# ishine/minimax-speech

Measured on AMD Instinct MI355X. Metric: 24 kHz audio-seconds generated per wall-second per node (CosyVoice2-0.5B-shaped LM + flow + DAC-VAE, end to end), higher is better.
Workload: dtype bf16

## Files before the change

include/mmx_hip_lab.h:

```cpp
#ifndef MMX_HIP_LAB_H
#define MMX_HIP_LAB_H
#ifdef __cplusplus
extern "C" {
#endif

int mmx_lab_skinny_stamps(void* buf);

int mmx_lab_tail_stamps(void* buf);

#ifdef __cplusplus
}
#endif
#endif
```

minimax-speech_amd/csrc/llm.hip:

```cpp
#include "common.h"
#include "../../include/mmx_hip.h"

template <typename T>
__global__ void pack_skinny_kernel(const T* __restrict__ w, long ldw, int N, int K, const float* __restrict__ kscale,
                                   int half, T* __restrict__ wp) {
    constexpr int E = sizeof(T) == 2 ? 8 : 4;
    constexpr int KB = E * 4;
    const long total = (long)((N + 15) / 16) * (K / KB) * 64 * E;
    for (long idx = (long)blockIdx.x * blockDim.x + threadIdx.x; idx < total; idx += (long)gridDim.x * blockDim.x) {
        int j = idx % E;
        long t = idx / E;
        int lane = t % 64;
        t /= 64;
        int kb = t % (K / KB);
        int tile = t / (K / KB);
        int col = lane & 15, g = lane >> 4;
        int row;
        if (half > 0) row = (tile & 1) * half + (tile >> 1) * 16 + col;
        else row = tile * 16 + col;
        int kk = kb * KB + g * E + j;
        float v = 0.f;
        if (row < N && (half == 0 || ((tile >> 1) * 16 + col) < half)) {
            v = Cvt<T>::to_f(w[(long)row * ldw + kk]);
            if (kscale) v *= kscale[kk];
// ... 343 lines not shown
                               const int32_t* __restrict__ block_table, int max_pages, int page) {
    constexpr int D = 64, HALF = 32;
    const int b = blockIdx.y, t = blockIdx.x;
    const int p = pos[b] + t;
    const float* src = qkv + (long)b * qkv_bs + (long)t * ldqkv;
    const int nh = Hq + 2 * Hkv;
    const int phys = block_table[(long)b * max_pages + p / page];
    const int slot = p % page;
    for (int i = threadIdx.x; i < nh * HALF; i += blockDim.x) {
        const int hh = i / HALF, d = i % HALF;
        const float x0 = src[hh * D + d], x1 = src[hh * D + d + HALF];
        float y0 = x0, y1 = x1;
        if (hh < Hq + Hkv) {
            const float ang = (float)p * inv_freq[d];
            const float c = cosf(ang), s = sinf(ang);
            y0 = x0 * c - x1 * s;
            y1 = x1 * c + x0 * s;
        }
        if (hh < Hq) {
            T* o = q_out + (long)b * q_bs + (long)t * ldq + hh * D;
            o[d] = Cvt<T>::from_f(y0);
            o[d + HALF] = Cvt<T>::from_f(y1);
        } else {
            const int hk = (hh - Hq) % Hkv;
            T* base = (hh < Hq + Hkv ? kc : vc) + (((long)phys * Hkv + hk) * page + slot) * D;
            base[d] = Cvt<T>::from_f(y0);
            base[d + HALF] = Cvt<T>::from_f(y1);
        }
    }
}
extern "C" int mmx_rope_kv_store(const float* qkv, int64_t ldqkv, int64_t qkv_bs, int B, int rows, int Hq, int Hkv, int D,
                                 const float* inv_freq, const int32_t* pos, void* q_out, int64_t ldq, int64_t q_bs,
                                 void* kc, void* vc, const int32_t* block_table, int max_pages, int page,
                                 int dtype, hipStream_t stream) {
    dtype = MMX_ACT_DTYPE(dtype);
    MMX_CHECK_ARG(qkv && inv_freq && pos && q_out && kc && vc && block_table && B > 0 && rows > 0 && D == 64 && page > 0);
    dim3 grid(rows, B);
    if (dtype == MMX_BF16) hipLaunchKernelGGL(rope_kv_kernel<bf16_t>, grid, dim3(256), 0, stream, qkv, ldqkv, qkv_bs, Hq, Hkv, inv_freq, pos, (bf16_t*)q_out, ldq, q_bs, (bf16_t*)kc, (bf16_t*)vc, block_table, max_pages, page);
    else if (dtype == MMX_F32) hipLaunchKernelGGL(rope_kv_kernel<float>, grid, dim3(256), 0, stream, qkv, ldqkv, qkv_bs, Hq, Hkv, inv_freq, pos, (float*)q_out, ldq, q_bs, (float*)kc, (float*)vc, block_table, max_pages, page);
    else return MMX_EARG;
    MMX_LAUNCH_CHECK();
    return MMX_OK;
}

template <typename T>
__global__ __launch_bounds__(256) void paged_attn_kernel(
    const T* __restrict__ q, long ldq, long q_bs, int Hq, int Hkv, float scale, const int32_t* __restrict__ pos,
    const T* __restrict__ kc, const T* __restrict__ vc, const int32_t* __restrict__ block_table, int max_pages,
    int page, T* __restrict__ out, long ldo, long o_bs) {
    constexpr int D = 64;
    extern __shared__ __attribute__((aligned(16))) char smem[];
    float* qs = reinterpret_cast<float*>(smem);
    float* red = qs + D;
    float* S = red + 8 + 4 * D;
    const int tid = threadIdx.x, lane = tid & 63, wave = tid >> 6;
    const int h = blockIdx.x, t = blockIdx.y, b = blockIdx.z;
    const int hk = h / (Hq / Hkv);
    const int ctx = pos[b] + t + 1;
    const int32_t* bt = block_table + (long)b * max_pages;
    if (tid < D) qs[tid] = Cvt<T>::to_f(q[(long)b * q_bs + (long)t * ldq + h * D + tid]);
    __syncthreads();
    float mx = -INFINITY;
    for (int j = tid; j < ctx; j += 256) {
        const T* kp = kc + (((long)bt[j / page] * Hkv + hk) * page + j % page) * D;
        float s = 0.f;
#pragma unroll
        for (int d = 0; d < D; ++d) s += qs[d] * Cvt<T>::to_f(kp[d]);
        s *= scale;
        S[j] = s;
        mx = fmaxf(mx, s);
    }
    mx = wave_max(mx);
    if (lane == 0) red[wave] = mx;
    __syncthreads();
    mx = fmaxf(fmaxf(red[0], red[1]), fmaxf(red[2], red[3]));
    float l = 0.f;
    for (int j = tid; j < ctx; j += 256) {
        float e = expf(S[j] - mx);
        S[j] = e;
        l += e;
    }
    l = wave_sum(l);
    if (lane == 0) red[4 + wave] = l;
    __syncthreads();
    l = red[4] + red[5] + red[6] + red[7];
    float acc = 0.f;
    for (int j = wave; j < ctx; j += 4) {
        const T* vp = vc + (((long)bt[j / page] * Hkv + hk) * page + j % page) * D;
        acc += S[j] * Cvt<T>::to_f(vp[lane]);
    }
    red[8 + wave * D + lane] = acc;
    __syncthreads();
    if (wave == 0) {
        float o = (red[8 + lane] + red[8 + D + lane]) + (red[8 + 2 * D + lane] + red[8 + 3 * D + lane]);
        out[(long)b * o_bs + (long)t * ldo + h * D + lane] = Cvt<T>::from_f(o / l);
    }
}
extern "C" int mmx_paged_attn(const void* q, int64_t ldq, int64_t q_bs, int B, int rows, int Hq, int Hkv, int D, float scale,
                              const int32_t* pos, const void* kc, const void* vc, const int32_t* block_table, int max_pages,
                              int page, void* out, int64_t ldo, int64_t o_bs, int dtype, hipStream_t stream) {
    dtype = MMX_ACT_DTYPE(dtype);
    MMX_CHECK_ARG(q && pos && kc && vc && block_table && out && B > 0 && rows > 0 && D == 64 && Hq % Hkv == 0 && page > 0);
    const size_t max_ctx = (size_t)max_pages * page;
    size_t lds = (64 + 8 + 4 * 64 + max_ctx) * 4;
    MMX_CHECK_ARG(lds <= 160 * 1024);
    dim3 grid(Hq, rows, B);
    if (dtype == MMX_BF16) MMX_LDS_OPT_IN(paged_attn_kernel<bf16_t>, lds);
    else if (dtype == MMX_F32) MMX_LDS_OPT_IN(paged_attn_kernel<float>, lds);
    if (dtype == MMX_BF16) hipLaunchKernelGGL(paged_attn_kernel<bf16_t>, grid, dim3(256), lds, stream, (const bf16_t*)q, ldq, q_bs, Hq, Hkv, scale, pos, (const bf16_t*)kc, (const bf16_t*)vc, block_table, max_pages, page, (bf16_t*)out, ldo, o_bs);
    else if (dtype == MMX_F32) hipLaunchKernelGGL(paged_attn_kernel<float>, grid, dim3(256), lds, stream, (const float*)q, ldq, q_bs, Hq, Hkv, scale, pos, (const float*)kc, (const float*)vc, block_table, max_pages, page, (float*)out, ldo, o_bs);
    else return MMX_EARG;
    MMX_LAUNCH_CHECK();
    return MMX_OK;
}

template <typename T>
__device__ __forceinline__ void load8(const T* p, float o[8]) {
    if constexpr (sizeof(T) == 2) {
        uint4 r = *reinterpret_cast<const uint4*>(p);
        const unsigned w[4] = {r.x, r.y, r.z, r.w};
#pragma unroll
        for (int i = 0; i < 4; ++i) {
            o[2 * i] = __uint_as_float(w[i] << 16);
            o[2 * i + 1] = __uint_as_float(w[i] & 0xffff0000u);
        }
    } else {
        float4 a = *reinterpret_cast<const float4*>(p), b = *reinterpret_cast<const float4*>(p + 4);
        o[0] = a.x; o[1] = a.y; o[2] = a.z; o[3] = a.w; o[4] = b.x; o[5] = b.y; o[6] = b.z; o[7] = b.w;
    }
}
template <typename T>
struct Raw8 {
    uint4 a, b;
    __device__ __forceinline__ void load(const T* p) {
        a = *reinterpret_cast<const uint4*>(p);
        if constexpr (sizeof(T) == 4) b = *reinterpret_cast<const uint4*>(p + 4);
    }
    __device__ __forceinline__ void to_float(float o[8]) const {
        const unsigned w[4] = {a.x, a.y, a.z, a.w};
        if constexpr (sizeof(T) == 2) {
#pragma unroll
            for (int i = 0; i < 4; ++i) {
                o[2 * i] = __uint_as_float(w[i] << 16);
                o[2 * i + 1] = __uint_as_float(w[i] & 0xffff0000u);
            }
        } else {
            const unsigned w2[4] = {b.x, b.y, b.z, b.w};
#pragma unroll
            for (int i = 0; i < 4; ++i) { o[i] = __uint_as_float(w[i]); o[4 + i] = __uint_as_float(w2[i]); }
        }
    }
};

template <typename T, int OM, int HP>
__global__ __launch_bounds__(256) void decode_attn_kernel(
    const float* __restrict__ qkv, long ldqkv, int Hq, int Hkv, const float* __restrict__ inv_freq,
    const float* __restrict__ rope_tab, const int32_t* __restrict__ pos, T* __restrict__ kc, T* __restrict__ vc,
    const int32_t* __restrict__ block_table, int max_pages, int page, float scale, T* __restrict__ out, long ldo,
    int nseq) {
    constexpr int D = 64, HALF = 32, NG = 32;
    extern __shared__ __attribute__((aligned(16))) char smem[];
    float* qs = reinterpret_cast<float*>(smem);
    float* kn = qs + HP * D;
    float* vn = kn + D;
    float* gm = vn + D;
    float* gl = gm + HP * NG;
    float* part = gl + HP * NG;
    int* bts = reinterpret_cast<int*>(part + HP * NG * D);
    const int tid = threadIdx.x;
    const int group = Hq / Hkv, nsub = (group + HP - 1) / HP;
    const int xcd = blockIdx.x & 7, slot = blockIdx.x >> 3;
    const int kvg = (slot / nsub) * 8 + xcd;
    if (kvg >= Hkv * nseq) return;
    const int b = kvg / Hkv, hk = kvg % Hkv, sub = slot % nsub;
    const int h0 = hk * group + sub * HP, nh = min(HP, group - sub * HP);
    const int32_t* bt = block_table + (long)b * max_pages;
    for (int i = tid; i < max_pages; i += 256) bts[i] = bt[i];
    const int p = pos[b];
    const float* src = qkv + (long)b * ldqkv;
    const float sc2 = scale * 1.44269504088896341f;
    if (tid < (HP + 1) * HALF) {
        const int which = tid >> 5, d = tid & 31;
        const float* x = src + (which < HP ? (h0 + min(which, nh - 1)) * D : (Hq + hk) * D);
        float c, s;
        if (rope_tab) {
            c = rope_tab[(long)p * D + d];
            s = rope_tab[(long)p * D + HALF + d];
        } else {
            const float ang = (float)p * inv_freq[d];
            c = cosf(ang);
            s = sinf(ang);
        }
        const float y0 = x[d] * c - x[d + HALF] * s, y1 = x[d + HALF] * c + x[d] * s;
        if (which < HP) { qs[which * D + d] = y0 * sc2; qs[which * D + d + HALF] = y1 * sc2; }
        else { kn[d] = Cvt<T>::to_f(Cvt<T>::from_f(y0)); kn[d + HALF] = Cvt<T>::to_f(Cvt<T>::from_f(y1)); }
    } else if (tid < (HP + 1) * HALF + D) {
        const int d = tid - (HP + 1) * HALF;
        vn[d] = Cvt<T>::to_f(Cvt<T>::from_f(src[(Hq + Hkv + hk) * D + d]));
    }
    __syncthreads();
    if (sub == 0 && tid < D) {
        const long o = (((long)bts[p / page] * Hkv + hk) * page + p % page) * D + tid;
        kc[o] = Cvt<T>::from_f(kn[tid]);
        vc[o] = Cvt<T>::from_f(vn[tid]);
    }
    const int kg = tid >> 3, dc = tid & 7;
    float qv[HP][8];
#pragma unroll
    for (int hp = 0; hp < HP; ++hp)
#pragma unroll
        for (int e = 0; e < 8; ++e) qv[hp][e] = qs[hp * D + dc * 8 + e];
    float m[HP], l[HP], acc[HP][8];
#pragma unroll
    for (int hp = 0; hp < HP; ++hp) {
        m[hp] = -INFINITY;
        l[hp] = 0.f;
#pragma unroll
        for (int e = 0; e < 8; ++e) acc[hp][e] = 0.f;
    }
    auto consume = [&](const float kv[8], const float vv[8]) {
#pragma unroll
        for (int hp = 0; hp < HP; ++hp) {
            float sdot = 0.f;
#pragma unroll
            for (int e = 0; e < 8; ++e) sdot = __builtin_fmaf(qv[hp][e], kv[e], sdot);
            sdot = group8_sum(sdot);
            const float mn = fmaxf(m[hp], sdot);
            const float al = __builtin_amdgcn_exp2f(m[hp] - mn), pj = __builtin_amdgcn_exp2f(sdot - mn);
            l[hp] = __builtin_fmaf(l[hp], al, pj);
#pragma unroll
            for (int e = 0; e < 8; ++e) acc[hp][e] = __builtin_fmaf(acc[hp][e], al, pj * vv[e]);
            m[hp] = mn;
        }
    };
    constexpr int U = sizeof(T) == 2 ? 12 : 10;
    for (int j0 = kg; j0 < p; j0 += NG * U) {
        Raw8<T> rk[U], rv[U];
#pragma unroll
        for (int u = 0; u < U; ++u) {
            const int j = j0 + u * NG;
            if (j < p) {
                const long o = (((long)bts[j / page] * Hkv + hk) * page + j % page) * D + dc * 8;
                rk[u].load(kc + o);
                rv[u].load(vc + o);
            }
        }
#pragma unroll
        for (int u = 0; u < U; ++u) {
            if (j0 + u * NG < p) {
                float kv[8], vv[8];
                rk[u].to_float(kv);
                rv[u].to_float(vv);
                consume(kv, vv);
            }
        }
    }
    if (kg == p % NG) {
        float kv[8], vv[8];
#pragma unroll
        for (int e = 0; e < 8; ++e) { kv[e] = kn[dc * 8 + e]; vv[e] = vn[dc * 8 + e]; }
        consume(kv, vv);
    }
#pragma unroll
    for (int hp = 0; hp < HP; ++hp) {
        if (dc == 0) { gm[hp * NG + kg] = m[hp]; gl[hp * NG + kg] = l[hp]; }
#pragma unroll
        for (int e = 0; e < 8; ++e) part[(hp * NG + kg) * D + dc * 8 + e] = acc[hp][e];
    }
    __syncthreads();
    if (tid < nh * D) {
        const int hp = tid >> 6, d = tid & 63, h = h0 + hp;
        const float* gmh = gm + hp * NG;
        const float* glh = gl + hp * NG;
        const float* ph = part + hp * NG * D;
        float M = -INFINITY;
#pragma unroll
        for (int g2 = 0; g2 < NG; ++g2) M = fmaxf(M, gmh[g2]);
        float L = 0.f, o = 0.f;
#pragma unroll
        for (int g2 = 0; g2 < NG; ++g2) {
            const float w = __builtin_amdgcn_exp2f(gmh[g2] - M);
            L = __builtin_fmaf(glh[g2], w, L);
            o = __builtin_fmaf(ph[g2 * D + d], w, o);
        }
        if constexpr (OM == 2) {
            const int nkb = Hq * D / 32, col = h * D + d;
            const long ps = (long)((nseq + 15) / 16) * nkb * 512;
            const long idx = ((((long)(b >> 4) * nkb + (col >> 5)) * 64) + (((col & 31) >> 3) << 4) + (b & 15)) * 8 + (col & 7);
            bf16_t* pl = reinterpret_cast<bf16_t*>(out);
            const float v = o / L;
            const bf16_t hh = f2bf(v);
            const float r1 = v - bf2f(hh);
            const bf16_t mm = f2bf(r1);
            pl[idx] = hh;
            pl[ps + idx] = mm;
            pl[2 * ps + idx] = f2bf(r1 - bf2f(mm));
        } else if constexpr (OM == 3) {
            const int nkb = Hq * D / 32, col = h * D + d;
            const long ps = (long)((nseq + 15) / 16) * nkb * 512;
            const long idx = ((((long)(b >> 4) * nkb + (col >> 5)) * 64) + (((col & 31) >> 3) << 4) + (b & 15)) * 8 + (col & 7);
            unsigned short* pl = reinterpret_cast<unsigned short*>(out);
            const float v = o / L;
            const _Float16 hh = (_Float16)v;
            pl[idx] = __builtin_bit_cast(unsigned short, hh);
            pl[ps + idx] = __builtin_bit_cast(unsigned short, (_Float16)(v - (float)hh));
        } else {
            out[OM == 1 ? act_packed_index<T>(b, h * D + d, Hq * D) : (long)b * ldo + h * D + d] = Cvt<T>::from_f(o / L);
        }
    }
}

template <bool OPK, int G>
__global__ __launch_bounds__(256) void decode_attn_gqa_kernel(
    const float* __restrict__ qkv, long ldqkv, int Hq, int Hkv, const float* __restrict__ inv_freq,
    const float* __restrict__ rope_tab, const int32_t* __restrict__ pos, bf16_t* __restrict__ kc, bf16_t* __restrict__ vc,
    const int32_t* __restrict__ block_table, int max_pages, float scale, bf16_t* __restrict__ out, long ldo, int nseq) {
    constexpr int D = 64, HALF = 32, PAGE = 16, NS = 8;
    static_assert(G <= 8, "one 8-float row of P per key");
    extern __shared__ __attribute__((aligned(16))) char smem[];
    bf16_t* qh = reinterpret_cast<bf16_t*>(smem);
    bf16_t* ql = qh + 16 * D;
    bf16_t* kn = ql + 16 * D;
    bf16_t* vn = kn + D;
    float* Pw = reinterpret_cast<float*>(vn + D);
    float* Aw = Pw + 4 * NS * 16 * 8;
    float* gm = Aw + 32;
    float* gl = gm + 32;
    float* part = gl + 32;
    int* bts = reinterpret_cast<int*>(part + 32 * G * D);
    const int tid = threadIdx.x, wave = tid >> 6, lane = tid & 63, l16 = lane & 15, g = lane >> 4;
    const int b = blockIdx.x / Hkv, hk = blockIdx.x % Hkv;
    const int32_t* bt = block_table + (long)b * max_pages;
    const int p = pos[b];
    const int NT = p / PAGE + 1;
    for (int i = tid; i < NT; i += 256) bts[i] = bt[i];
    for (int i = tid; i < 2 * 16 * D / 2; i += 256) reinterpret_cast<unsigned*>(qh)[i] = 0u;
    __syncthreads();
    const float* src = qkv + (long)b * ldqkv;
    const float sc2 = scale * 1.44269504088896341f;
    {
        const int which = tid >> 5, d = tid & 31;
        if (which <= G) {
            const float* x = src + (which < G ? (hk * G + which) * D : (Hq + hk) * D);
            float c, s;
            if (rope_tab) {
                c = rope_tab[(long)p * D + d];
                s = rope_tab[(long)p * D + HALF + d];
            } else {
                const float ang = (float)p * inv_freq[d];
                c = cosf(ang);
                s = sinf(ang);
            }
            const float y0 = x[d] * c - x[d + HALF] * s, y1 = x[d + HALF] * c + x[d] * s;
            if (which < G) {
                const float a0 = y0 * sc2, a1 = y1 * sc2;
                const bf16_t h0 = f2bf(a0), h1 = f2bf(a1);
                qh[which * D + d] = h0;
                qh[which * D + d + HALF] = h1;
                ql[which * D + d] = f2bf(a0 - bf2f(h0));
                ql[which * D + d + HALF] = f2bf(a1 - bf2f(h1));
            } else {
                kn[d] = f2bf(y0);
                kn[d + HALF] = f2bf(y1);
            }
        }
        if (tid < D) vn[tid] = f2bf(src[(Hq + Hkv + hk) * D + tid]);
    }
    __syncthreads();
    if (tid < D) {
        const long o = (((long)bts[p / PAGE] * Hkv + hk) * PAGE + p % PAGE) * D + tid;
        kc[o] = kn[tid];
        vc[o] = vn[tid];
    }
    short8_t bqh[2], bql[2];
#pragma unroll
    for (int ks = 0; ks < 2; ++ks) {
        bqh[ks] = *reinterpret_cast<const short8_t*>(qh + l16 * D + ks * 32 + 8 * g);
        bql[ks] = *reinterpret_cast<const short8_t*>(ql + l16 * D + ks * 32 + 8 * g);
    }
    const int ksub = lane >> 3, dc = lane & 7;
    const int tp = p / PAGE, rp = p % PAGE;
    float* Pme = Pw + wave * NS * 16 * 8;
    float m_run = -INFINITY, l_part = 0.f;
    typedef __attribute__((ext_vector_type(2))) float float2_t;
    float2_t acc[G][4];
#pragma unroll
    for (int h = 0; h < G; ++h)
#pragma unroll
        for (int e = 0; e < 4; ++e) acc[h][e] = float2_t{0.f, 0.f};

    for (int r0 = 0; r0 < NT; r0 += 4 * NS) {
        if (r0 + wave >= NT) break;
        uint4 rk[NS][2], rv[NS][2];
#pragma unroll
        for (int i = 0; i < NS; ++i) {
            const int t = r0 + 4 * i + wave;
            if (t < NT) {
                const long base = ((long)bts[t] * Hkv + hk) * PAGE * D;
#pragma unroll
                for (int ks = 0; ks < 2; ++ks) rk[i][ks] = *reinterpret_cast<const uint4*>(kc + base + l16 * D + ks * 32 + 8 * g);
#pragma unroll
                for (int hf = 0; hf < 2; ++hf) rv[i][hf] = *reinterpret_cast<const uint4*>(vc + base + (ksub + 8 * hf) * D + dc * 8);
            }
        }
        float4_t sacc[NS];
        float bm = -INFINITY;
#pragma unroll
        for (int i = 0; i < NS; ++i) {
            const int t = r0 + 4 * i + wave;
            sacc[i] = float4_t{-INFINITY, -INFINITY, -INFINITY, -INFINITY};
            if (t < NT) {
                if (t == tp) {
                    if (l16 == rp) {
#pragma unroll
                        for (int ks = 0; ks < 2; ++ks) rk[i][ks] = *reinterpret_cast<const uint4*>(kn + ks * 32 + 8 * g);
                    }
#pragma unroll
                    for (int hf = 0; hf < 2; ++hf) {
                        if (ksub + 8 * hf == rp) rv[i][hf] = *reinterpret_cast<const uint4*>(vn + dc * 8);
                        if (ksub + 8 * hf > rp) rv[i][hf] = make_uint4(0u, 0u, 0u, 0u);
                    }
                }
                float4_t c = {0.f, 0.f, 0.f, 0.f};
#pragma unroll
                for (int ks = 0; ks < 2; ++ks) {
                    const short8_t ak = __builtin_bit_cast(short8_t, rk[i][ks]);
                    c = __builtin_amdgcn_mfma_f32_16x16x32_bf16(ak, bqh[ks], c, 0, 0, 0);
                    c = __builtin_amdgcn_mfma_f32_16x16x32_bf16(ak, bql[ks], c, 0, 0, 0);
                }
#pragma unroll
                for (int r = 0; r < 4; ++r) {
                    const float x = (t * PAGE + 4 * g + r <= p) ? c[r] : -INFINITY;
                    sacc[i][r] = x;
                    bm = fmaxf(bm, x);
                }
            }
        }
        bm = fmaxf(bm, __shfl_xor(bm, 16, 64));
        bm = fmaxf(bm, __shfl_xor(bm, 32, 64));
        const float m_new = fmaxf(m_run, bm);
        const float alpha = __builtin_amdgcn_exp2f(m_run - m_new);
        m_run = m_new;
        float rs = 0.f;
#pragma unroll
        for (int i = 0; i < NS; ++i) {
            if (r0 + 4 * i + wave < NT) {
#pragma unroll
                for (int r = 0; r < 4; ++r) {
                    const float pj = __builtin_amdgcn_exp2f(sacc[i][r] - m_new);
                    rs += pj;
                    if (l16 < 8) Pme[(i * 16 + 4 * g + r) * 8 + l16] = pj;
                }
            }
        }
        l_part = l_part * alpha + rs;
        if (l16 < 8 && g == 0) Aw[wave * 8 + l16] = alpha;
        __builtin_amdgcn_fence(__ATOMIC_RELEASE, "wavefront");
        __builtin_amdgcn_wave_barrier();
        {
            const float4 a0 = *reinterpret_cast<const float4*>(Aw + wave * 8), a1 = *reinterpret_cast<const float4*>(Aw + wave * 8 + 4);
            const float al[8] = {a0.x, a0.y, a0.z, a0.w, a1.x, a1.y, a1.z, a1.w};
#pragma unroll
            for (int h = 0; h < G; ++h)
#pragma unroll
                for (int e = 0; e < 4; ++e) acc[h][e] *= al[h];
        }
#pragma unroll
        for (int i = 0; i < NS; ++i) {
            if (r0 + 4 * i + wave < NT) {
#pragma unroll
                for (int hf = 0; hf < 2; ++hf) {
                    const float* pr = Pme + (i * 16 + ksub + 8 * hf) * 8;
                    const float4 p0 = *reinterpret_cast<const float4*>(pr), p1 = *reinterpret_cast<const float4*>(pr + 4);
                    const float pv[8] = {p0.x, p0.y, p0.z, p0.w, p1.x, p1.y, p1.z, p1.w};
                    const unsigned w[4] = {rv[i][hf].x, rv[i][hf].y, rv[i][hf].z, rv[i][hf].w};
                    float2_t vv[4];
#pragma unroll
                    for (int e = 0; e < 4; ++e) vv[e] = float2_t{__uint_as_float(w[e] << 16), __uint_as_float(w[e] & 0xffff0000u)};
#pragma unroll
                    for (int h = 0; h < G; ++h) {
                        const float2_t ph = {pv[h], pv[h]};
#pragma unroll
                        for (int e = 0; e < 4; ++e) acc[h][e] = __builtin_elementwise_fma(ph, vv[e], acc[h][e]);
                    }
                }
            }
        }
        __builtin_amdgcn_fence(__ATOMIC_RELEASE, "wavefront");
        __builtin_amdgcn_wave_barrier();
    }
    l_part += __shfl_xor(l_part, 16, 64);
    l_part += __shfl_xor(l_part, 32, 64);
    if (l16 < 8 && g == 0) { gm[wave * 8 + l16] = m_run; gl[wave * 8 + l16] = l_part; }
#pragma unroll
    for (int h = 0; h < G; ++h) {
        float* pp = part + ((long)(wave * 8 + ksub) * G + h) * D + dc * 8;
        *reinterpret_cast<float4*>(pp) = make_float4(acc[h][0].x, acc[h][0].y, acc[h][1].x, acc[h][1].y);
        *reinterpret_cast<float4*>(pp + 4) = make_float4(acc[h][2].x, acc[h][2].y, acc[h][3].x, acc[h][3].y);
    }
    __syncthreads();
    for (int idx = tid; idx < G * D; idx += 256) {
        const int h = idx / D, d = idx % D;
        float M = -INFINITY;
#pragma unroll
        for (int w = 0; w < 4; ++w) M = fmaxf(M, gm[w * 8 + h]);
        float L = 0.f, o = 0.f;
#pragma unroll
        for (int w = 0; w < 4; ++w) {
            const float wt = __builtin_amdgcn_exp2f(gm[w * 8 + h] - M);
            L += gl[w * 8 + h] * wt;
            float sacc2 = 0.f;
#pragma unroll
            for (int k2 = 0; k2 < 8; ++k2) sacc2 += part[((long)(w * 8 + k2) * G + h) * D + d];
            o += sacc2 * wt;
        }
        const int col = (hk * G + h) * D + d;
        out[OPK ? act_packed_index<bf16_t>(b, col, Hq * D) : (long)b * ldo + col] = f2bf(o / L);
    }
}
extern "C" int mmx_decode_attn(const float* qkv, int64_t ldqkv, int B, int Hq, int Hkv, int D, const float* inv_freq,
                               const float* rope_tab, const int32_t* pos, void* kc, void* vc, const int32_t* block_table, int max_pages,
                               int page, float scale, void* out, int64_t ldo, int dtype, int out_packed, hipStream_t stream) {
    dtype = MMX_ACT_DTYPE(dtype);
    MMX_CHECK_ARG(qkv && (inv_freq || rope_tab) && pos && kc && vc && block_table && out && B > 0 && D == 64 && Hq % Hkv == 0 && page > 0);
    MMX_CHECK_ARG(out_packed >= 0 && out_packed <= 31);
    const bool gqa_shared = !(out_packed & 2);
    const bool split_out = out_packed & 4;
    const bool split_h2 = out_packed & 8;
    const bool one_head = (out_packed & 16) || (long)B * Hq <= 256;
    MMX_CHECK_ARG(!(split_out || split_h2) || (dtype == MMX_F32 && !(out_packed & 1) && !(split_out && split_h2)));
    out_packed &= 1;
    const size_t max_ctx = (size_t)max_pages * page;
    (void)max_ctx;
    const int hp = one_head ? 1 : 2, nsub = (Hq / Hkv + hp - 1) / hp;
    size_t lds = ((size_t)hp * 64 + 2 * 64 + 2 * hp * 32 + (size_t)hp * 32 * 64 + (size_t)max_pages) * 4;
    MMX_CHECK_ARG(lds <= 64 * 1024);
    dim3 grid(8 * ((Hkv * B + 7) / 8) * nsub);
#define DA(T, OM) do { if (one_head) hipLaunchKernelGGL((decode_attn_kernel<T, OM, 1>), grid, dim3(256), lds, stream, qkv, ldqkv, Hq, Hkv, inv_freq, rope_tab, pos, (T*)kc, (T*)vc, block_table, max_pages, page, scale, (T*)out, ldo, B); \
                       else hipLaunchKernelGGL((decode_attn_kernel<T, OM, 2>), grid, dim3(256), lds, stream, qkv, ldqkv, Hq, Hkv, inv_freq, rope_tab, pos, (T*)kc, (T*)vc, block_table, max_pages, page, scale, (T*)out, ldo, B); } while (0)
    if (dtype == MMX_BF16 && page == 16 && Hq == 7 * Hkv && gqa_shared) {
        const size_t lds2 = (2 * 16 * 64 + 2 * 64) * 2 + (4 * 8 * 16 * 8 + 3 * 32 + 32 * 7 * 64 + (size_t)max_pages) * 4;
        MMX_CHECK_ARG(lds2 <= 160 * 1024);
        if (out_packed) MMX_LDS_OPT_IN((decode_attn_gqa_kernel<true, 7>), lds2);
        else MMX_LDS_OPT_IN((decode_attn_gqa_kernel<false, 7>), lds2);
#define DG(OPK) hipLaunchKernelGGL((decode_attn_gqa_kernel<OPK, 7>), dim3(Hkv * B), dim3(256), lds2, stream, qkv, ldqkv, Hq, Hkv, inv_freq, rope_tab, pos, (bf16_t*)kc, (bf16_t*)vc, block_table, max_pages, scale, (bf16_t*)out, ldo, B)
        if (out_packed) DG(true); else DG(false);
    } else if (dtype == MMX_BF16) { if (out_packed) DA(bf16_t, 1); else DA(bf16_t, 0); }
    else if (dtype == MMX_F32) { if (split_h2) DA(float, 3); else if (split_out) DA(float, 2); else if (out_packed) DA(float, 1); else DA(float, 0); }
    else return MMX_EARG;
    MMX_LAUNCH_CHECK();
    return MMX_OK;
}
```

minimax-speech_amd/mmx/ops.py:

```python
import ctypes as C
import math

import torch

from . import _lib as L
from ._lib import ACT, BF16, F32, check, i64, load, stream, _p


def round_up(x, m):
    return (x + m - 1) // m * m


class Planed(torch.Tensor):
    """A packed weight held as bf16 PLANES hi + [mid +] lo = w of an fp32 checkpoint's values (include/mmx_hip.h MMX_X2W / MMX_X3W).
    The type is the marker: gemm() / skinny2() switch to the weight-plane dtype code when they are handed one; views and row
    slices keep the type (torch's default __torch_function__)."""


def weight_planes(w: torch.Tensor, n: int):
    out, r = [], w.float()
    for _ in range(n):
        t = r.to(torch.bfloat16)
        out.append(t)
        r = r - t.float()
# ... 259 lines not shown
                                   _p(pos_u), _p(pos_v), _p(out), i64(ldo), i64(o_bs), B, H, T, C.c_float(scale), chunk, _p(klen), stream()),
          "mmx_attn_relpos_x")


def attn_flash_bf16(q, k, vt, out, *, B, H, T, ldq, ldk, ldvt, ldo, q_bs, k_bs, vt_bs, o_bs, scale, keymask=None,
                    chunk=0, q_begin=0, km_bs=None, fp8=False, klen=None):
    if klen is not None:
        assert klen.dtype == torch.int32 and klen.numel() >= B
    if fp8:
        check(load().mmx_attn_flash_fp8(_p(q), i64(ldq), i64(q_bs), _p(k), i64(ldk), i64(k_bs), _p(vt), i64(ldvt),
                                        i64(vt_bs), _p(out), i64(ldo), i64(o_bs), B, H, T, C.c_float(scale),
                                        _p(keymask), i64(T if km_bs is None else km_bs), chunk, q_begin, _p(klen), stream()), "mmx_attn_flash_fp8")
        return
    check(load().mmx_attn_flash_bf16(_p(q), i64(ldq), i64(q_bs), _p(k), i64(ldk), i64(k_bs), _p(vt), i64(ldvt),
                                     i64(vt_bs), _p(out), i64(ldo), i64(o_bs), B, H, T, C.c_float(scale),
                                     _p(keymask), i64(T if km_bs is None else km_bs), chunk, q_begin, _p(klen), stream()), "mmx_attn_flash_bf16")


def attn_flash_x(q, k, v, out, *, B, H, T, ldq, ldk, ldv, ldo, q_bs, k_bs, v_bs, o_bs, scale, keymask=None, chunk=0, q_begin=0,
                 km_bs=None, klen=None):
    if klen is not None:
        assert klen.dtype == torch.int32 and klen.numel() >= B
    check(load().mmx_attn_flash_x(_p(q), i64(ldq), i64(q_bs), _p(k), i64(ldk), i64(k_bs), _p(v), i64(ldv), i64(v_bs),
                                  _p(out), i64(ldo), i64(o_bs), B, H, T, C.c_float(scale), _p(keymask),
                                  i64(T if km_bs is None else km_bs), chunk, q_begin, _p(klen), stream()), "mmx_attn_flash_x")


def attn_flash_xs(qk, vt, out, *, B, H, T, ldqk, ldvt, ldo, qk_bs, vt_bs, o_bs, scale, keymask=None, chunk=0, q_begin=0, km_bs=None,
                  klen=None, form=0):
    if klen is not None:
        assert klen.dtype == torch.int32 and klen.numel() >= B
    check(load().mmx_attn_flash_xs(_p(qk), i64(ldqk), i64(qk_bs), _p(vt), i64(ldvt), i64(vt_bs), _p(out), i64(ldo), i64(o_bs), B, H, T,
                                   C.c_float(scale), _p(keymask), i64(T if km_bs is None else km_bs), chunk, q_begin, _p(klen), int(form),
                                   stream()), "mmx_attn_flash_xs")


def pack_skinny(w, *, dtype, kscale=None, interleave_half=0):
    N, K = w.shape
    if dtype in L.WPLANES:
        assert w.dtype == torch.float32 and kscale is None
        base = {L.X2W: L.X2, L.X3W: L.X3}[dtype]
        return torch.cat([pack_skinny(t.contiguous(), dtype=base, interleave_half=interleave_half)
                          for t in weight_planes(w, L.WPLANES[dtype])]).as_subclass(Planed)
    assert w.dtype == L.WEIGHT_DT[dtype]
    KB = 32 if L.WEIGHT_DT[dtype] == torch.bfloat16 else 16
    tiles = (N + 15) // 16
    wp = torch.empty(tiles * (K // KB) * 64 * (KB // 4), dtype=L.WEIGHT_DT[dtype], device=w.device)
    check(load().mmx_pack_skinny(_p(w), i64(w.stride(0)), N, K, _p(kscale), interleave_half, _p(wp), dtype, stream()),
          "mmx_pack_skinny")
    return wp


X_PACKED, OUT_PACKED = 1, 2


def packed_rows(B):
    return (B + 15) // 16 * 16


def pack_act(x, dtype):
    E = 8 if dtype == BF16 else 4
    B, K = x.shape
    R = packed_rows(B)
    xp = torch.zeros(R, K, dtype=x.dtype, device=x.device)
    xp[:B] = x
    return xp.reshape(R // 16, 16, K // (4 * E), 4, E).permute(0, 2, 3, 1, 4).contiguous().reshape(-1)


def unpack_act(xp, B, K, dtype):
    E = 8 if dtype == BF16 else 4
    R = packed_rows(B)
    return xp.reshape(R // 16, K // (4 * E), 4, 16, E).permute(0, 3, 1, 2, 4).reshape(R, K)[:B]


def skinny_gemm(x, wp, *, B, K, N, dtype, bias=None, rs=False, eps=1e-6, epi=0, out_f32=None, out_act=None,
                ldx=None, ldo_f=None, ldo_a=None, x_packed=False, out_packed=False, kgamma=None):
    xdt = L.dt_of(x)
    flags = (X_PACKED if x_packed else 0) | (OUT_PACKED if out_packed else 0)
    check(load().mmx_skinny_gemm(_p(x), xdt, i64(ldx if ldx is not None else K), B, K, N, _p(wp), _p(bias), int(rs),
                                 C.c_float(eps), epi, _p(out_f32), i64(ldo_f if ldo_f is not None else N),
                                 _p(out_act), i64(ldo_a if ldo_a is not None else N), dtype, flags, _p(kgamma), stream()),
          "mmx_skinny_gemm")


SSQ_SLOTS = 64


def plane_elems(B, K):
    return packed_rows(B) * K


def split_planes(x, f16=False):
    B, K = x.shape
    out, r = [], x.float()
    for _ in range(2 if f16 else 3):
        t = r.to(torch.float16 if f16 else torch.bfloat16)
        out.append(pack_act(t.view(torch.bfloat16) if f16 else t, BF16))
        r = r - t.float()
    return torch.stack(out)


def merge_planes(xs, B, K, f16=False):
    if f16:
        return sum(unpack_act(xs[s], B, K, BF16).contiguous().view(torch.float16).float() for s in range(2))
    return sum(unpack_act(xs[s], B, K, BF16).float() for s in range(3))


H2_WSCALE = 256.0


def pack_skinny_h2(w, *, planes=1, interleave_half=0):
    ws = w.float() * H2_WSCALE
    assert float(ws.abs().max()) < 65504.0, "weight out of the fp16 range of MMX_H2"
    out, r = [], ws
    for _ in range(planes):
        t = r.to(torch.float16)
        out.append(pack_skinny(t.view(torch.bfloat16).contiguous(), dtype=L.X3, interleave_half=interleave_half))
        r = r - t.float()
    return out[0] if planes == 1 else torch.cat(out).as_subclass(Planed)


def decode_prep(x, xs, ssq, *, B, K, gamma=None, h=None, dtype=L.X3):
    check(load().mmx_decode_prep(_p(x), i64(x.shape[-1]), B, K, _p(gamma), _p(h), i64(h.shape[-1] if h is not None else 0), _p(xs),
                                 _p(ssq), dtype, stream()), "mmx_decode_prep")


def skinny2(xs, wp, *, B, K, N, dtype, bias=None, ssq_in=None, eps=1e-6, epi=0, out=None, ldo=None, xs_out=None, gamma_next=None,
            ssq_out=None, tiles_per_wg=1, ksplit=1, part=None, tickets=None):
    if isinstance(wp, Planed):
        dtype = L.H2W if dtype in (L.H2, L.H2W) else L.X3W
    check(load().mmx_skinny2(_p(xs), B, K, N, _p(wp), _p(bias), _p(ssq_in), C.c_float(eps), epi, _p(out),
                             i64(ldo if ldo is not None else N), _p(xs_out), _p(gamma_next), _p(ssq_out), tiles_per_wg, ksplit,
                             _p(part), i64(part.numel() if part is not None else 0), _p(tickets), dtype, stream()), "mmx_skinny2")


def rope_kv_store(qkv, inv_freq, pos, q_out, kc, vc, block_table, *, B, rows, Hq, Hkv, page, dtype, ldqkv=None, qkv_bs=None,
                  ldq=None, q_bs=None):
    ldqkv = (Hq + 2 * Hkv) * 64 if ldqkv is None else ldqkv
    ldq = Hq * 64 if ldq is None else ldq
    check(load().mmx_rope_kv_store(_p(qkv), i64(ldqkv), i64(rows * ldqkv if qkv_bs is None else qkv_bs), B, rows, Hq, Hkv, 64,
                                   _p(inv_freq), _p(pos), _p(q_out), i64(ldq), i64(rows * ldq if q_bs is None else q_bs), _p(kc), _p(vc),
                                   _p(block_table), block_table.shape[1], page, dtype, stream()), "mmx_rope_kv_store")


def paged_attn(q, pos, kc, vc, block_table, out, *, B, rows, Hq, Hkv, page, dtype, ldq=None, q_bs=None, ldo=None, o_bs=None):
    ldq = Hq * 64 if ldq is None else ldq
    ldo = Hq * 64 if ldo is None else ldo
    check(load().mmx_paged_attn(_p(q), i64(ldq), i64(rows * ldq if q_bs is None else q_bs), B, rows, Hq, Hkv, 64, C.c_float(0.125),
                                _p(pos), _p(kc), _p(vc), _p(block_table), block_table.shape[1], page, _p(out),
                                i64(ldo), i64(rows * ldo if o_bs is None else o_bs), dtype, stream()), "mmx_paged_attn")


def decode_attn(qkv, inv_freq, pos, kc, vc, block_table, out, *, B, Hq, Hkv, page, dtype, rope_tab=None, out_packed=False,
                per_head=False, out_split=False, one_head=False, ldqkv=None, ldo=None):
    check(load().mmx_decode_attn(_p(qkv), i64((Hq + 2 * Hkv) * 64 if ldqkv is None else ldqkv), B, Hq, Hkv, 64, _p(inv_freq), _p(rope_tab),
                                 _p(pos), _p(kc), _p(vc), _p(block_table), block_table.shape[1], page, C.c_float(0.125), _p(out),
                                 i64(Hq * 64 if ldo is None else ldo), dtype, int(bool(out_packed)) | (2 if per_head else 0) | (8 if out_split == "f16" else (4 if out_split else 0)) | (16 if one_head else 0), stream()), "mmx_decode_attn")


def swiglu(gu, out, *, rows, I, dtype, ldgu=None, ldo=None):
    check(load().mmx_swiglu(_p(gu), i64(ldgu or 2 * I), rows, I, _p(out), i64(ldo or I), dtype, stream()), "mmx_swiglu")


def sample_step(logits, state, out_tokens, speech_emb, next_x, *, V, B, eos_id, seed, top_k=25, top_p=0.8,
                win_size=10, tau_r=0.1, sampled=None, forced=None, logp_out=None):
    check(load().mmx_sample_step(_p(logits), i64(logits.shape[-1]), V, B, eos_id, top_k, C.c_float(top_p), win_size,
                                 C.c_float(tau_r), C.c_uint64(seed), _p(state), _p(out_tokens), out_tokens.shape[1],
                                 _p(sampled), _p(forced), _p(speech_emb), speech_emb.shape[1], _p(next_x),
                                 i64(next_x.shape[-1]), _p(logp_out), stream()), "mmx_sample_step")


SAMP_MODE, SAMP_TOP_K, SAMP_WIN, SAMP_TOP_P, SAMP_TAU_R, SAMP_SEED_LO, SAMP_SEED_HI = range(7)
SAMPLER_MODES = {"ras": 0, "nucleus": 1, "random": 2}


def sampler_column(mode=0, top_p=0.8, top_k=25, win_size=10, tau_r=0.1, seed=0):
    import struct
    mode = SAMPLER_MODES.get(mode, mode)
    if mode not in (0, 1, 2) or not 1 <= int(top_k) <= 64 or not 0 <= int(win_size) <= 64:
        raise ValueError(f"sampler out of range: mode {mode!r} (0..2), top_k {top_k} (1..64), win_size {win_size} (0..64)")
    bits = lambda v: struct.unpack("<i", struct.pack("<f", float(v)))[0]
    i32 = lambda u: u - (1 << 32) if u >= (1 << 31) else u
    seed = int(seed) & ((1 << 64) - 1)
    return [int(mode), int(top_k), int(win_size), bits(top_p), bits(tau_r), i32(seed & 0xffffffff), i32(seed >> 32), 0]


def sample_step_tab(logits, state, out_tokens, speech_emb, next_x, samp, *, V, B, eos_id, sampled=None, forced=None, logp_out=None):
    assert samp.dtype == torch.int32 and samp.is_contiguous() and samp.shape == (8, B)
    check(load().mmx_sample_step_tab(_p(logits), i64(logits.shape[-1]), V, B, eos_id, _p(samp), _p(state), _p(out_tokens),
                                     out_tokens.shape[1], _p(sampled), _p(forced), _p(speech_emb), speech_emb.shape[1],
                                     _p(next_x), i64(next_x.shape[-1]), _p(logp_out), stream()), "mmx_sample_step_tab")
```

Measured before the change: 554.0.

## Prefetch paged KV ahead of RoPE prologue and pipeline loads in decode attention

The decode attention kernel now issues the first KV-cache loads before the RoPE/q-staging prologue and its barrier. It then runs a rolling software pipeline that refills each register slot right after consuming it, instead of load-all-then-consume passes. The aim is to hide global-memory latency for the paged K/V reads and overlap them with the prologue. Out-of-range slots load from a dummy address. The old order stays available behind a flag, and lab-only timestamp instrumentation is added, at the cost of more register pressure and code complexity.

Measured after the change: 559.1, median of 6. About the same (+0.9%).

```diff
diff --git a/include/mmx_hip_lab.h b/include/mmx_hip_lab.h
--- a/include/mmx_hip_lab.h
+++ b/include/mmx_hip_lab.h
@@ -8,6 +8,10 @@
 
 int mmx_lab_tail_stamps(void* buf);
 
+int mmx_lab_dattn_stamps(void* buf);
+
+int mmx_lab_dattn_one_head_max(int bhq);
+
 #ifdef __cplusplus
 }
 #endif
diff --git a/minimax-speech_amd/csrc/llm.hip b/minimax-speech_amd/csrc/llm.hip
--- a/minimax-speech_amd/csrc/llm.hip
+++ b/minimax-speech_amd/csrc/llm.hip
@@ -519,7 +519,15 @@
     }
 };
 
-template <typename T, int OM, int HP>
+#ifndef MMX_DATTN_EARLY
+#define MMX_DATTN_EARLY 2
+#endif
+#ifndef MMX_DATTN_FILL
+#define MMX_DATTN_FILL 4
+#endif
+__device__ unsigned long long* g_dattn_stamps = nullptr;
+#define DSTAMP(i) do { if constexpr (LAB) ts[(i)] = __builtin_amdgcn_s_memtime(); } while (0)
+template <typename T, int OM, int HP, bool LEG>
 __global__ __launch_bounds__(256) void decode_attn_kernel(
     const float* __restrict__ qkv, long ldqkv, int Hq, int Hkv, const float* __restrict__ inv_freq,
     const float* __restrict__ rope_tab, const int32_t* __restrict__ pos, T* __restrict__ kc, T* __restrict__ vc,
@@ -542,36 +550,94 @@
     const int b = kvg / Hkv, hk = kvg % Hkv, sub = slot % nsub;
     const int h0 = hk * group + sub * HP, nh = min(HP, group - sub * HP);
     const int32_t* bt = block_table + (long)b * max_pages;
-    for (int i = tid; i < max_pages; i += 256) bts[i] = bt[i];
-    const int p = pos[b];
     const float* src = qkv + (long)b * ldqkv;
     const float sc2 = scale * 1.44269504088896341f;
-    if (tid < (HP + 1) * HALF) {
-        const int which = tid >> 5, d = tid & 31;
-        const float* x = src + (which < HP ? (h0 + min(which, nh - 1)) * D : (Hq + hk) * D);
-        float c, s;
-        if (rope_tab) {
-            c = rope_tab[(long)p * D + d];
-            s = rope_tab[(long)p * D + HALF + d];
-        } else {
+    const int kg = tid >> 3, dc = tid & 7;
+    constexpr int U = sizeof(T) == 2 ? 12 : 10;
+    constexpr int F = MMX_DATTN_FILL < U ? MMX_DATTN_FILL : U;
+    constexpr int E = MMX_DATTN_EARLY < F ? MMX_DATTN_EARLY : F;
+    Raw8<T> rk[U], rv[U];
+    unsigned long long ts[10] = {};
+    DSTAMP(0);
+    int p;
+    const T* idle = reinterpret_cast<const T*>(src) + dc * 8;
+    const int qstep = NG / page, rstep = NG % page;
+    int jn = kg, qn = kg / page, rn = kg % page;
+    auto request = [&](int u, int pg) {
+        const long o = (((long)pg * Hkv + hk) * page + rn) * D + dc * 8;
+        rk[u].load(jn < p ? kc + o : idle);
+        rv[u].load(jn < p ? vc + o : idle);
+        jn += NG;
+        qn += qstep;
+        rn += rstep;
+        if (rn >= page) { rn -= page; ++qn; }
+    };
+    if constexpr (LEG) {
+        for (int i = tid; i < max_pages; i += 256) bts[i] = bt[i];
+        p = pos[b];
+        if (tid < (HP + 1) * HALF) {
+            const int which = tid >> 5, d = tid & 31;
+            const float* x = src + (which < HP ? (h0 + min(which, nh - 1)) * D : (Hq + hk) * D);
+            float c, s;
+            if (rope_tab) {
+                c = rope_tab[(long)p * D + d];
+                s = rope_tab[(long)p * D + HALF + d];
+            } else {
+                const float ang = (float)p * inv_freq[d];
+                c = cosf(ang);
+                s = sinf(ang);
+            }
+            const float y0 = x[d] * c - x[d + HALF] * s, y1 = x[d + HALF] * c + x[d] * s;
+            if (which < HP) { qs[which * D + d] = y0 * sc2; qs[which * D + d + HALF] = y1 * sc2; }
+            else { kn[d] = Cvt<T>::to_f(Cvt<T>::from_f(y0)); kn[d + HALF] = Cvt<T>::to_f(Cvt<T>::from_f(y1)); }
+        } else if (tid < (HP + 1) * HALF + D) {
+            const int d = tid - (HP + 1) * HALF;
+            vn[d] = Cvt<T>::to_f(Cvt<T>::from_f(src[(Hq + Hkv + hk) * D + d]));
+        }
+        DSTAMP(1);
+        __syncthreads();
+    } else {
+        p = pos[b];
+        int pg[E > 0 ? E : 1];
+        {
+            int q = qn, r = rn;
+#pragma unroll
+            for (int u = 0; u < E; ++u) {
+                pg[u] = bt[min(q, max_pages - 1)];
+                q += qstep;
+                r += rstep;
+                if (r >= page) { r -= page; ++q; }
+            }
+        }
+        const int bt0 = bt[min(tid, max_pages - 1)];
+        const int role = tid >> 5, d = tid & 31;
+        const float* x = src + (role < HP ? (h0 + min(role, nh - 1)) * D : role == HP ? (Hq + hk) * D
+                                                                                      : (Hq + Hkv + hk) * D + (role == HP + 2 ? HALF : 0));
+        const float x0 = x[d], x1 = x[role <= HP ? d + HALF : d];
+        const float* rt = rope_tab ? rope_tab + (long)p * D : src;
+        float c = rt[d], sn = rt[HALF + d];
+#pragma unroll
+        for (int u = 0; u < E; ++u) request(u, pg[u]);
+        if (!rope_tab) {
             const float ang = (float)p * inv_freq[d];
             c = cosf(ang);
-            s = sinf(ang);
-        }
-        const float y0 = x[d] * c - x[d + HALF] * s, y1 = x[d + HALF] * c + x[d] * s;
-        if (which < HP) { qs[which * D + d] = y0 * sc2; qs[which * D + d + HALF] = y1 * sc2; }
-        else { kn[d] = Cvt<T>::to_f(Cvt<T>::from_f(y0)); kn[d + HALF] = Cvt<T>::to_f(Cvt<T>::from_f(y1)); }
-    } else if (tid < (HP + 1) * HALF + D) {
-        const int d = tid - (HP + 1) * HALF;
-        vn[d] = Cvt<T>::to_f(Cvt<T>::from_f(src[(Hq + Hkv + hk) * D + d]));
-    }
-    __syncthreads();
+            sn = sinf(ang);
+        }
+        const float y0 = x0 * c - x1 * sn, y1 = x1 * c + x0 * sn;
+        if (role < HP) { qs[role * D + d] = y0 * sc2; qs[role * D + d + HALF] = y1 * sc2; }
+        else if (role == HP) { kn[d] = Cvt<T>::to_f(Cvt<T>::from_f(y0)); kn[d + HALF] = Cvt<T>::to_f(Cvt<T>::from_f(y1)); }
+        else if (role <= HP + 2) vn[(role - HP - 1) * HALF + d] = Cvt<T>::to_f(Cvt<T>::from_f(x0));
+        if (tid < max_pages) bts[tid] = bt0;
+        for (int i = tid + 256; i < max_pages; i += 256) bts[i] = bt[i];
+        DSTAMP(1);
+        __syncthreads();
+    }
+    DSTAMP(2);
     if (sub == 0 && tid < D) {
         const long o = (((long)bts[p / page] * Hkv + hk) * page + p % page) * D + tid;
         kc[o] = Cvt<T>::from_f(kn[tid]);
         vc[o] = Cvt<T>::from_f(vn[tid]);
     }
-    const int kg = tid >> 3, dc = tid & 7;
     float qv[HP][8];
 #pragma unroll
     for (int hp = 0; hp < HP; ++hp)
@@ -600,27 +666,57 @@
             m[hp] = mn;
         }
     };
-    constexpr int U = sizeof(T) == 2 ? 12 : 10;
-    for (int j0 = kg; j0 < p; j0 += NG * U) {
-        Raw8<T> rk[U], rv[U];
-#pragma unroll
-        for (int u = 0; u < U; ++u) {
-            const int j = j0 + u * NG;
-            if (j < p) {
-                const long o = (((long)bts[j / page] * Hkv + hk) * page + j % page) * D + dc * 8;
-                rk[u].load(kc + o);
-                rv[u].load(vc + o);
-            }
-        }
-#pragma unroll
-        for (int u = 0; u < U; ++u) {
-            if (j0 + u * NG < p) {
-                float kv[8], vv[8];
-                rk[u].to_float(kv);
-                rv[u].to_float(vv);
-                consume(kv, vv);
-            }
-        }
+    auto consume_slot = [&](int u, int j) {
+        if (j < p) {
+            float kv[8], vv[8];
+            rk[u].to_float(kv);
+            rv[u].to_float(vv);
+            consume(kv, vv);
+        }
+    };
+    if constexpr (LEG) {
+        int pass = 0;
+        for (int j0 = kg; j0 < p; j0 += NG * U, ++pass) {
+#pragma unroll
+            for (int u = 0; u < U; ++u) {
+                const int j = j0 + u * NG;
+                if (j < p) {
+                    const long o = (((long)bts[j / page] * Hkv + hk) * page + j % page) * D + dc * 8;
+                    rk[u].load(kc + o);
+                    rv[u].load(vc + o);
+                }
+            }
+#pragma unroll
+            for (int u = 0; u < U; ++u) {
+                consume_slot(u, j0 + u * NG);
+                if (u == 0 && pass == 0) DSTAMP(3);
+            }
+            if (pass == 0) DSTAMP(4);
+            if (pass == 1) DSTAMP(5);
+        }
+    } else {
+#pragma unroll
+        for (int u = E; u < F; ++u) request(u, bts[min(qn, max_pages - 1)]);
+        int t = 0;
+        for (; (t * U + F) * NG < p; ++t) {
+            const int j0 = kg + t * (NG * U);
+#pragma unroll
+            for (int u = 0; u < U; ++u) {
+                consume_slot(u, j0 + u * NG);
+                request((u + F) % U, bts[min(qn, max_pages - 1)]);
+                if (u == 0 && t == 0) DSTAMP(3);
+            }
+            if (t == 0) DSTAMP(4);
+            if (t == 1) DSTAMP(5);
+        }
+        const int j0 = kg + t * (NG * U);
+#pragma unroll
+        for (int u = 0; u < F; ++u) {
+            consume_slot(u, j0 + u * NG);
+            if (u == 0 && t == 0) DSTAMP(3);
+        }
+        if (t == 0) DSTAMP(4);
+        if (t == 1) DSTAMP(5);
     }
     if (kg == p % NG) {
         float kv[8], vv[8];
@@ -628,6 +724,7 @@
         for (int e = 0; e < 8; ++e) { kv[e] = kn[dc * 8 + e]; vv[e] = vn[dc * 8 + e]; }
         consume(kv, vv);
     }
+    DSTAMP(6);
 #pragma unroll
     for (int hp = 0; hp < HP; ++hp) {
         if (dc == 0) { gm[hp * NG + kg] = m[hp]; gl[hp * NG + kg] = l[hp]; }
@@ -635,6 +732,7 @@
         for (int e = 0; e < 8; ++e) part[(hp * NG + kg) * D + dc * 8 + e] = acc[hp][e];
     }
     __syncthreads();
+    DSTAMP(7);
     if (tid < nh * D) {
         const int hp = tid >> 6, d = tid & 63, h = h0 + hp;
         const float* gmh = gm + hp * NG;
@@ -675,7 +773,18 @@
             out[OM == 1 ? act_packed_index<T>(b, h * D + d, Hq * D) : (long)b * ldo + h * D + d] = Cvt<T>::from_f(o / L);
         }
     }
-}
+    if constexpr (LAB) {
+        unsigned long long* st = g_dattn_stamps;
+        if (st) {
+            asm volatile("s_waitcnt vmcnt(0)" ::: "memory");
+            DSTAMP(8);
+            if ((tid & 63) == 0)
+#pragma unroll
+                for (int i = 0; i < 9; ++i) st[((long)blockIdx.x * 4 + (tid >> 6)) * 16 + i] = ts[i];
+        }
+    }
+}
+#undef DSTAMP
 
 template <bool OPK, int G>
 __global__ __launch_bounds__(256) void decode_attn_gqa_kernel(
@@ -885,16 +994,22 @@
         out[OPK ? act_packed_index<bf16_t>(b, col, Hq * D) : (long)b * ldo + col] = f2bf(o / L);
     }
 }
+#if MMX_LAB
+static int one_head_max = 256;
+#else
+constexpr int one_head_max = 256;
+#endif
 extern "C" int mmx_decode_attn(const float* qkv, int64_t ldqkv, int B, int Hq, int Hkv, int D, const float* inv_freq,
                                const float* rope_tab, const int32_t* pos, void* kc, void* vc, const int32_t* block_table, int max_pages,
                                int page, float scale, void* out, int64_t ldo, int dtype, int out_packed, hipStream_t stream) {
     dtype = MMX_ACT_DTYPE(dtype);
     MMX_CHECK_ARG(qkv && (inv_freq || rope_tab) && pos && kc && vc && block_table && out && B > 0 && D == 64 && Hq % Hkv == 0 && page > 0);
-    MMX_CHECK_ARG(out_packed >= 0 && out_packed <= 31);
+    MMX_CHECK_ARG(out_packed >= 0 && out_packed <= 63);
     const bool gqa_shared = !(out_packed & 2);
     const bool split_out = out_packed & 4;
     const bool split_h2 = out_packed & 8;
-    const bool one_head = (out_packed & 16) || (long)B * Hq <= 256;
+    const bool one_head = (out_packed & 16) || (long)B * Hq <= one_head_max;
+    const bool legacy = out_packed & 32;
     MMX_CHECK_ARG(!(split_out || split_h2) || (dtype == MMX_F32 && !(out_packed & 1) && !(split_out && split_h2)));
     out_packed &= 1;
     const size_t max_ctx = (size_t)max_pages * page;
@@ -903,8 +1018,9 @@
     size_t lds = ((size_t)hp * 64 + 2 * 64 + 2 * hp * 32 + (size_t)hp * 32 * 64 + (size_t)max_pages) * 4;
     MMX_CHECK_ARG(lds <= 64 * 1024);
     dim3 grid(8 * ((Hkv * B + 7) / 8) * nsub);
-#define DA(T, OM) do { if (one_head) hipLaunchKernelGGL((decode_attn_kernel<T, OM, 1>), grid, dim3(256), lds, stream, qkv, ldqkv, Hq, Hkv, inv_freq, rope_tab, pos, (T*)kc, (T*)vc, block_table, max_pages, page, scale, (T*)out, ldo, B); \
-                       else hipLaunchKernelGGL((decode_attn_kernel<T, OM, 2>), grid, dim3(256), lds, stream, qkv, ldqkv, Hq, Hkv, inv_freq, rope_tab, pos, (T*)kc, (T*)vc, block_table, max_pages, page, scale, (T*)out, ldo, B); } while (0)
+#define DA3(T, OM, HP_, LEG_) hipLaunchKernelGGL((decode_attn_kernel<T, OM, HP_, LEG_>), grid, dim3(256), lds, stream, qkv, ldqkv, Hq, Hkv, inv_freq, rope_tab, pos, (T*)kc, (T*)vc, block_table, max_pages, page, scale, (T*)out, ldo, B)
+#define DA(T, OM) do { if (one_head) { if (legacy) DA3(T, OM, 1, true); else DA3(T, OM, 1, false); } \
+                       else { if (legacy) DA3(T, OM, 2, true); else DA3(T, OM, 2, false); } } while (0)
     if (dtype == MMX_BF16 && page == 16 && Hq == 7 * Hkv && gqa_shared) {
         const size_t lds2 = (2 * 16 * 64 + 2 * 64) * 2 + (4 * 8 * 16 * 8 + 3 * 32 + 32 * 7 * 64 + (size_t)max_pages) * 4;
         MMX_CHECK_ARG(lds2 <= 160 * 1024);
@@ -918,3 +1034,15 @@
     MMX_LAUNCH_CHECK();
     return MMX_OK;
 }
+
+#if MMX_LAB
+extern "C" int mmx_lab_dattn_stamps(void* buf) {
+    unsigned long long* p = reinterpret_cast<unsigned long long*>(buf);
+    const hipError_t e = hipMemcpyToSymbol(HIP_SYMBOL(g_dattn_stamps), &p, sizeof(p));
+    return e == hipSuccess ? MMX_OK : -(int)e - 1000;
+}
+extern "C" int mmx_lab_dattn_one_head_max(int bhq) {
+    one_head_max = bhq;
+    return MMX_OK;
+}
+#endif
diff --git a/minimax-speech_amd/mmx/ops.py b/minimax-speech_amd/mmx/ops.py
--- a/minimax-speech_amd/mmx/ops.py
+++ b/minimax-speech_amd/mmx/ops.py
@@ -435,10 +435,10 @@
 
 
 def decode_attn(qkv, inv_freq, pos, kc, vc, block_table, out, *, B, Hq, Hkv, page, dtype, rope_tab=None, out_packed=False,
-                per_head=False, out_split=False, one_head=False, ldqkv=None, ldo=None):
+                per_head=False, out_split=False, one_head=False, legacy_order=False, ldqkv=None, ldo=None):
     check(load().mmx_decode_attn(_p(qkv), i64((Hq + 2 * Hkv) * 64 if ldqkv is None else ldqkv), B, Hq, Hkv, 64, _p(inv_freq), _p(rope_tab),
                                  _p(pos), _p(kc), _p(vc), _p(block_table), block_table.shape[1], page, C.c_float(0.125), _p(out),
-                                 i64(Hq * 64 if ldo is None else ldo), dtype, int(bool(out_packed)) | (2 if per_head else 0) | (8 if out_split == "f16" else (4 if out_split else 0)) | (16 if one_head else 0), stream()), "mmx_decode_attn")
+                                 i64(Hq * 64 if ldo is None else ldo), dtype, int(bool(out_packed)) | (2 if per_head else 0) | (8 if out_split == "f16" else (4 if out_split else 0)) | (16 if one_head else 0) | (32 if legacy_order else 0), stream()), "mmx_decode_attn")
 
 
 def swiglu(gu, out, *, rows, I, dtype, ldgu=None, ldo=None):
```
